# allanbrondum/tfhe-aes-2

Measured on AMD Instinct MI355X. Metric: FHE AES-128 blocks/sec, higher is better.
Workload: dtype f64

## Files before the change

### tfhe-aes-2_amd/csrc/br512x4.hpp

```cpp
#pragma once
#include "br512.hpp"
#include "lf512.hpp"

namespace tae {
namespace br512x4 {

using br512::K1;
using br512::lds_sync;
using br512::M;
using br512::N;
using br512::swap16;
using br512::swap32;
using br512::u32x4;
using br512::wave_sync;

constexpr int C = 3, JOBS = C * K1, THREADS = 1024;

constexpr int BUF_STRIDE = 290;
__device__ constexpr int SF[16] = {-36, -45, -39, -38, -37, -30, -44, -31, -22, -55, -29, -20, -47, -28, -14, -53};
constexpr int SG1[4] = {42, 78, 74, 46};
constexpr int SG3[4] = {13, 81, 157, 225};
__host__ __device__ constexpr int sidx(int q) { return SF[4 * (q & 3) + ((q >> 4) & 3)] + SG1[(q >> 2) & 3] + SG3[q >> 6]; }

#define PRIO(n) __builtin_amdgcn_s_setprio(n)

#ifdef TAE_X4_PROF
#define PROF_DECL uint64_t prof_[10] = {0}, prof_t_ = clock64();
#define PROF_T(i)                        \
    do {                                 \
        asm volatile("" ::: "memory");   \
        const uint64_t now_ = clock64(); \
        prof_[i] += now_ - prof_t_;      \
        prof_t_ = now_;                  \
    } while (0)
#else
#define PROF_DECL
#define PROF_T(i) \
    do {          \
    } while (0)
#endif

constexpr int ACC_STRIDE = N;

#ifdef TAE_X4_HALFTW
__device__ __forceinline__ cplx twmul(cplx a, cplx b) { return {fma(a.re, b.re, a.im), fma(a.im, b.im, a.re)}; }
#else
__device__ __forceinline__ cplx twmul(cplx a, cplx b) { return cmul(a, b); }
#endif

template <bool INV>
__device__ __forceinline__ void dft16x4(cplx *v, const cplx *tw) {
    dft4<INV>(v[0], v[1], v[2], v[3]);
    v[1] = twmul(v[1], INV ? cconj(tw[0]) : tw[0]);
    v[2] = twmul(v[2], INV ? cconj(tw[1]) : tw[1]);
    v[3] = twmul(v[3], INV ? cconj(tw[2]) : tw[2]);
#ifndef TAE_X4_NOSWAP
    swap32(v[0], v[2]);
    swap32(v[1], v[3]);
    swap16(v[0], v[1]);
    swap16(v[2], v[3]);
#endif
    dft4<INV>(v[0], v[1], v[2], v[3]);
}

template <int G>
__device__ __forceinline__ void mac_level(const cplx *buf, int pos, cplx *accr, const cplx *gv) {
    constexpr int PI0 = 4 * G, NA = (15 - PI0) < 4 ? (15 - PI0) : 4, Q0 = PI0 / 3;
#pragma unroll
    for (int p = 0; p < K1; p++) {
        if (p == 2) PRIO(2);
        if (p == 3) PRIO(1);
        if (p == 4) PRIO(0);
        cplx x[C];
#pragma unroll
        for (int c = 0; c < C; c++) x[c] = buf[(c * K1 + p) * BUF_STRIDE + pos];
#pragma unroll
        for (int a = 0; a < NA; a++) {
            const int pi = PI0 + a, q = pi / 3, c = pi % 3;
            const cplx gg = gv[p * 2 + (q - Q0)];
            double re = accr[a].re, im = accr[a].im;
            re = fma(x[c].re, gg.re, re);
            re = fma(-x[c].im, gg.im, re);
            im = fma(x[c].re, gg.im, im);
            im = fma(x[c].im, gg.re, im);
            accr[a] = {re, im};
        }
    }
}

template <int G>
__device__ __forceinline__ void mac_store(cplx *buf, int pos, const cplx *accr) {
    constexpr int PI0 = 4 * G, NA = (15 - PI0) < 4 ? (15 - PI0) : 4;
#pragma unroll
    for (int a = 0; a < NA; a++) {
        const int pi = PI0 + a, q = pi / 3, c = pi % 3;
        buf[(c * K1 + q) * BUF_STRIDE + pos] = accr[a];
    }
}

template <int LEV, bool PBS, int BLOG>
__global__ void __launch_bounds__(THREADS, 1)
    br_kernel(const uint64_t *__restrict__ lwe_in, int n, const uint64_t *__restrict__ lut, int n_out,
              const cplx *__restrict__ ggsw_base, int n_in, uint64_t *__restrict__ out, long B,
              uint64_t body_add, uint64_t out_add, const cplx *__restrict__ twist, const cplx *__restrict__ wtab,
              const double *__restrict__ lf, uint64_t *__restrict__ clk, long lut_mod = 1) {
    constexpr int LOGN = 9;
    ClockStamp stamp;
    stamp.start(clk);
    extern __shared__ __align__(16) unsigned char smem[];
    uint64_t *acc = reinterpret_cast<uint64_t *>(smem);
    cplx *buf = reinterpret_cast<cplx *>(acc + JOBS * ACC_STRIDE);
    cplx *s_tw = buf + JOBS * BUF_STRIDE;
    cplx *s_twa = s_tw + M;
    cplx *s_utw = s_twa + M;
    cplx *s_w16 = s_utw + M;
    double *s_lf = reinterpret_cast<double *>(s_tw);
    const cplx *s_untw = reinterpret_cast<const cplx *>(s_lf + lf512::UNTW);
    const int tid = threadIdx.x;
    const int jb = __builtin_amdgcn_readfirstlane(tid >> 6);
    const int lane = tid & 63, u = lane & 15, r = lane >> 4;
    const bool fjob = jb < JOBS;
    const int jct = fjob ? jb / K1 : 0;
    const size_t ggsw_sz = (size_t)LEV * K1 * K1 * M;

    long ct0, g = 0;
    int nct;
    if (PBS) {
        ct0 = (long)blockIdx.x * C;
        nct = (int)min((long)C, B - ct0);
    } else {
        const int nwg = (int)gridDim.x, q8 = nwg >> 3, r8 = nwg & 7, x8 = (int)blockIdx.x & 7;
        const int lb = x8 * q8 + min(x8, r8) + ((int)blockIdx.x >> 3);
        const int per_group = (n_out + C - 1) / C;
        g = lb / per_group;
        ct0 = (long)(lb - g * per_group) * C;
        nct = min(C, n_out - (int)ct0);
    }
    const bool jvalid = fjob && jct < nct;

    if constexpr (PBS) {
        for (int t = tid; t < lf512::KERNEL_DOUBLES; t += THREADS) s_lf[t] = lf[t];
    } else {
        for (int t = tid; t < M; t += THREADS) {
            s_tw[t] = twist[t];
            s_twa[t] = wtab[(t >> 4) * (t & 15)];
            s_utw[t] = cplx{twist[t].re * 0x1p-8, -twist[t].im * 0x1p-8};
        }
    }
    double lf_s2 = 0, lf_c8 = 0, lf_t8 = 0;
    if constexpr (PBS) {
        lf_s2 = lf[lf512::CONSTS];
        lf_c8 = lf[lf512::CONSTS + 1];
        lf_t8 = lf[lf512::CONSTS + 2];
    }
    if (!PBS && tid < 12) {
        const int rr = tid / 3, k1 = tid - 3 * rr + 1;
        const int e = (rr * k1) & 15;
        const cplx w = wtab[16 * e];
        s_w16[tid] = e == 0 ? cplx{1.0, 0.0} : (e == 4 ? cplx{0.0, -1.0} : w);
    }

    const cplx *gbase = PBS ? ggsw_base : ggsw_base + (size_t)g * n_in * ggsw_sz;
    const uint32_t gbytes = (uint32_t)((size_t)(PBS ? n : n_in) * ggsw_sz * sizeof(cplx));
    const __amdgpu_buffer_rsrc_t grs = __builtin_amdgcn_make_buffer_rsrc((void *)gbase, (short)0, gbytes, 0x00020000);
    const int grp = jb >> 2;
    const int pos = tid & (M - 1);
    const int gvoff = pos * (int)sizeof(cplx);
    const int spos = sidx(pos);
    const int baseA = SF[4 * (u & 3) + r] + SG1[u >> 2], baseB = SF[4 * r + (u & 3)] + SG3[u >> 2];
    const int q0 = (4 * grp) / 3;
    const int nq = grp == 3 ? 1 : 2;

    for (int t = tid; t < JOBS * N; t += THREADS) {
        const int job = t / N, j = t - job * N;
        const int ct = job / K1, c = job - ct * K1;
        uint64_t v = 0;
        if (ct < nct) {
            if (PBS) {
                const uint64_t *in = lwe_in + (size_t)(ct0 + ct) * (n + 1);
                const int bt = mod_switch(in[n] + body_add, LOGN);
                const int e0 = (2 * N - (bt % (2 * N))) % (2 * N);
                v = rotated_coeff(lut + ((ct0 + ct) % lut_mod) * (K1 * N) + c * N, j, e0, N);
            } else {
                v = c < K1 - 1 ? 0 : lut[(size_t)(ct0 + ct) * N + j];
            }
        }
        acc[job * ACC_STRIDE + j] = v;
    }
    lds_sync();

    const int steps = PBS ? n : n_in;
    uint64_t a_next = (PBS && jvalid) ? lwe_in[(size_t)(ct0 + jct) * (n + 1)] : 0;
    cplx accr[4];
    cplx gv[K1 * 2];
    const cplx *my_w16 = s_w16 + 3 * r;
    cplx *jbuf = buf + jb * BUF_STRIDE;
    PROF_DECL
    for (int step = 0; step < steps; step++) {
        int e, gstep;
        if (PBS) {
            const uint64_t a = a_next;
            if (step + 1 < steps && jvalid) a_next = lwe_in[(size_t)(ct0 + jct) * (n + 1) + step + 1];
            e = mod_switch(a, LOGN) % (2 * N);
            gstep = step * (int)(ggsw_sz * sizeof(cplx));
        } else {
            const int b = n_in - 1 - step;
            e = 2 * N - (1 << step);
            gstep = b * (int)(ggsw_sz * sizeof(cplx));
        }
        auto load_level = [&](int lev) {
#pragma unroll
            for (int p = 0; p < K1; p++)
#pragma unroll
                for (int qq = 0; qq < 2; qq++) {
                    if (qq < nq) {
                        const int soff = gstep + (((lev - 1) * K1 + p) * K1 + q0 + qq) * M * (int)sizeof(cplx);
                        const u32x4 rv = __builtin_amdgcn_raw_buffer_load_b128(grs, gvoff, soff, 0);
                        __builtin_memcpy(&gv[p * 2 + qq], &rv, sizeof(cplx));
                    }
                }
        };
        PRIO(3);
        int ll = lane;
        asm volatile("" : "+v"(ll));
        constexpr bool DBYTES = PBS && LEV > 3 && BLOG <= 7;
        uint32_t dig[DBYTES ? (LEV + 1) / 2 : LEV][4];
        constexpr bool FASTDEC = PBS && 128 * LEV * 8 <= (1 << BLOG);
        if (fjob) {
            const uint64_t *poly = acc + jb * ACC_STRIDE;
#pragma unroll
            for (int i = 0; i < 4; i++) {
                const int j = ll + 64 * i;
                uint64_t x0, x1;
                rot_diff<LOGN>(poly, j, e, poly[j], poly[j + M], x0, x1);
                uint32_t dp[LEV];
#ifdef TAE_X4_NODEC
#pragma unroll
                for (int l = 0; l < LEV; l++) dp[l] = (uint32_t)(x0 >> (20 * l)) ^ (uint32_t)(x1 >> (20 * l + 8));
#else
                if constexpr (FASTDEC) {
                    bool dok;
                    decompose16p_fast<LEV, BLOG>(x0, x1, dp, dok);
                    if (__builtin_amdgcn_ballot_w64(!dok)) decompose16p<LEV, BLOG>(x0, x1, dp);
                } else {
                    decompose16p<LEV, BLOG>(x0, x1, dp);
                }
#endif
                if constexpr (DBYTES) {
#pragma unroll
                    for (int l = 0; l < LEV; l += 2) {
                        const uint32_t up = l + 1 < LEV ? dp[(l + 1) % LEV] : 0u;
                        dig[l >> 1][i] = __builtin_amdgcn_perm(up, dp[l], 0x06040200u);
                    }
                } else {
#pragma unroll
                    for (int l = 0; l < LEV; l++) dig[l][i] = dp[l];
                }
            }
        }
#pragma unroll
        for (int a = 0; a < 4; a++) accr[a] = cplx{0.0, 0.0};
        PRIO(2);
        PROF_T(0);

#pragma unroll
        for (int lev = LEV; lev >= 1; lev--) {
            load_level(lev);
            if constexpr (PBS) {
                if (fjob) {
                    cplx v[4];
                    if constexpr (DBYTES) {
                        const int sh = ((lev - 1) & 1) * 16;
                        int dr[4], di[4];
#pragma unroll
                        for (int i = 0; i < 4; i++) {
                            uint32_t dw = dig[0][i];
#pragma unroll
                            for (int w = 1; w < (LEV + 1) / 2; w++)
                                if ((lev - 1) >> 1 == w) dw = dig[w][i];
                            dr[i] = __builtin_amdgcn_sbfe((int)dw, sh, 8);
                            di[i] = __builtin_amdgcn_sbfe((int)dw, sh + 8, 8);
                        }
                        lf512::a1i(dr, di, v, lf_s2, lf_c8, lf_t8);
                    } else {
                        uint32_t dw[4];
#pragma unroll
                        for (int i = 0; i < 4; i++) {
                            dw[i] = dig[0][i];
#pragma unroll
                            for (int l = 1; l < LEV; l++)
                                if (lev - 1 == l) dw[i] = dig[l][i];
                        }
                        lf512::a1(dw, v, lf_s2, lf_c8, lf_t8);
                    }
                    br512::transpose4(v);
                    lf512::dft4<false>(v, lf512::k4(s_lf, lf512::FA2, 4, r));
                    if (lev == LEV) PRIO(2);
#pragma unroll
                    for (int k2 = 0; k2 < 4; k2++) jbuf[baseA + SG3[k2]] = v[k2];
                }
                wave_sync();
                PRIO(1);
                PROF_T(1);
                if (fjob) {
                    cplx v[4];
#pragma unroll
                    for (int i = 0; i < 4; i++) v[i] = jbuf[baseB + SG1[i]];
                    lf512::dft4<false>(v, lf512::k4(s_lf, lf512::FB1, 16, u));
                    br512::transpose4(v);
                    lf512::dft4<false>(v, lf512::k4(s_lf, lf512::FB2, 64, lane));
                    PRIO(0);
#pragma unroll
                    for (int k2 = 0; k2 < 4; k2++) jbuf[baseB + SG1[k2]] = v[k2];
                }
            } else {
            cplx w16[3];
#pragma unroll
            for (int k = 0; k < 3; k++) w16[k] = my_w16[k];
            if (fjob) {
                cplx v[4];
#pragma unroll
                for (int i = 0; i < 4; i++) {
                    uint32_t dw = dig[0][i];
#pragma unroll
                    for (int l = 1; l < LEV; l++)
                        if (lev - 1 == l) dw = dig[l][i];
                    const double a0 = br512::lo16(dw), a1 = br512::hi16(dw);
                    const cplx tw = s_tw[ll + 64 * i];
#ifdef TAE_X4_HALFTW
                    v[i] = {fma(a0, tw.re, a1), fma(a1, tw.im, a0)};
#else
                    v[i] = {fma(a0, tw.re, -(a1 * tw.im)), fma(a0, tw.im, a1 * tw.re)};
#endif
                }
                dft16x4<false>(v, w16);
                if (lev == LEV) PRIO(2);
#pragma unroll
                for (int k2 = 0; k2 < 4; k2++) {
                    const int k = r + 4 * k2;
                    jbuf[baseA + SG3[k2]] = twmul(v[k2], s_twa[16 * k + u]);
                }
            }
            wave_sync();
            PRIO(1);
            PROF_T(1);
            if (fjob) {
                cplx v[4];
#pragma unroll
                for (int i = 0; i < 4; i++) v[i] = jbuf[baseB + SG1[i]];
                dft16x4<false>(v, w16);
                PRIO(0);
#pragma unroll
                for (int k2 = 0; k2 < 4; k2++) jbuf[baseB + SG1[k2]] = v[k2];
            }
            }
            PROF_T(2);
#ifdef TAE_X4_NOBARF
            asm volatile("s_waitcnt lgkmcnt(0)" ::: "memory");
#else
            lds_sync();
#endif
            PROF_T(3);
            PRIO(3);
            switch (grp) {
            case 0: mac_level<0>(buf, spos, accr, gv); break;
            case 1: mac_level<1>(buf, spos, accr, gv); break;
            case 2: mac_level<2>(buf, spos, accr, gv); break;
            default: mac_level<3>(buf, spos, accr, gv); break;
            }
            PROF_T(4);
#ifdef TAE_X4_NOBARM
            if (lev == 1) lds_sync();
#else
            lds_sync();
#endif
            PROF_T(5);
            PRIO(3);
        }
        switch (grp) {
        case 0: mac_store<0>(buf, spos, accr); break;
        case 1: mac_store<1>(buf, spos, accr); break;
        case 2: mac_store<2>(buf, spos, accr); break;
        default: mac_store<3>(buf, spos, accr); break;
        }
        lds_sync();
        PROF_T(6);
        PRIO(3);
        if constexpr (PBS) {
            if (fjob) {
                cplx v[4];
#pragma unroll
                for (int i = 0; i < 4; i++) v[i] = jbuf[baseB + SG1[i]];
                dft4<true>(v[0], v[1], v[2], v[3]);
                br512::transpose4(v);
                lf512::dft4<true>(v, lf512::k4(s_lf, lf512::IB2, 4, r));
#pragma unroll
                for (int k2 = 0; k2 < 4; k2++) jbuf[baseB + SG1[k2]] = v[k2];
            }
            wave_sync();
            PROF_T(7);
            PRIO(3);
            if (fjob) {
                cplx v[4];
#pragma unroll
                for (int i = 0; i < 4; i++) v[i] = jbuf[baseA + SG3[i]];
                lf512::dft4<true>(v, lf512::k4(s_lf, lf512::IA1, 16, u));
                br512::transpose4(v);
                lf512::dft4<true>(v, lf512::k4(s_lf, lf512::IA2, 64, lane));
                uint64_t *poly = acc + jb * ACC_STRIDE;
#pragma unroll
                for (int k2 = 0; k2 < 4; k2++) {
                    const int j = ll + 64 * k2;
                    const cplx t = cmul(v[k2], s_untw[j]);
#ifdef TAE_X4_NOTORUS
                    uint64_t a0 = poly[j] + f64_bits(t.re), a1 = poly[j + M] + f64_bits(t.im);
#else
                    bool o0, o1;
                    uint64_t a0 = torus_add_fast2_sh<8>(t.re, poly[j], o0), a1 = torus_add_fast2_sh<8>(t.im, poly[j + M], o1);
                    if (__builtin_amdgcn_ballot_w64(!(o0 && o1))) {
                        a0 = poly[j] + from_torus_bits(t.re * 0x1p-8);
                        a1 = poly[j + M] + from_torus_bits(t.im * 0x1p-8);
                    }
#endif
                    poly[j] = a0;
                    poly[j + M] = a1;
                }
            }
        } else {
        cplx w16[3];
#pragma unroll
        for (int k = 0; k < 3; k++) w16[k] = my_w16[k];
        if (fjob) {
            cplx v[4];
#pragma unroll
            for (int i = 0; i < 4; i++) v[i] = jbuf[baseB + SG1[i]];
            dft16x4<true>(v, w16);
#pragma unroll
            for (int k2 = 0; k2 < 4; k2++) jbuf[baseB + SG1[k2]] = v[k2];
        }
        wave_sync();
        PROF_T(7);
        PRIO(3);
        if (fjob) {
            cplx v[4];
#pragma unroll
            for (int i = 0; i < 4; i++) {
                const int kk = r + 4 * i;
                v[i] = twmul(jbuf[baseA + SG3[i]], cconj(s_twa[16 * kk + u]));
            }
            dft16x4<true>(v, w16);
            uint64_t *poly = acc + jb * ACC_STRIDE;
#pragma unroll
            for (int k2 = 0; k2 < 4; k2++) {
                const int j = ll + 64 * k2;
                const cplx t = twmul(v[k2], s_utw[j]);
                bool o0, o1;
                uint64_t a0 = torus_add_fast(t.re, poly[j], o0), a1 = torus_add_fast(t.im, poly[j + M], o1);
                if (__builtin_amdgcn_ballot_w64(!(o0 && o1))) {
                    a0 = poly[j] + from_torus_bits(t.re);
                    a1 = poly[j + M] + from_torus_bits(t.im);
                }
                poly[j] = a0;
                poly[j + M] = a1;
            }
        }
        }
        wave_sync();
        PROF_T(8);
#ifdef TAE_X4_PROF
        asm volatile("s_waitcnt lgkmcnt(0)" ::: "memory");
#endif
        PROF_T(9);
    }
#ifdef TAE_X4_PROF
    if (blockIdx.x == 100 && lane == 0)
        printf("x4prof wave %2d: dec %llu passA %llu passB %llu barF %llu mac %llu barM %llu store %llu invB %llu invA %llu end %llu\n",
               jb, (unsigned long long)prof_[0], (unsigned long long)prof_[1], (unsigned long long)prof_[2],
               (unsigned long long)prof_[3], (unsigned long long)prof_[4], (unsigned long long)prof_[5],
               (unsigned long long)prof_[6], (unsigned long long)prof_[7], (unsigned long long)prof_[8],
               (unsigned long long)prof_[9]);
#endif
    lds_sync();
    for (int ct = 0; ct < nct; ct++) {
        const uint64_t *a = acc + ct * K1 * ACC_STRIDE;
        uint64_t *o = PBS ? out + (size_t)(ct0 + ct) * (K1 - 1) * N + (size_t)(ct0 + ct)
                          : out + ((size_t)g * n_out + ct0 + ct) * ((K1 - 1) * N + 1);
        for (int t = tid; t < (K1 - 1) * N; t += THREADS) {
            const int p = t / N, j = t - p * N;
            o[t] = j == 0 ? a[p * ACC_STRIDE] : (0 - a[p * ACC_STRIDE + N - j]);
        }
        if (tid == 0) o[(K1 - 1) * N] = a[(K1 - 1) * ACC_STRIDE] + out_add;
    }
    stamp.stop(clk);
}

inline size_t lds_bytes() {
    return (size_t)JOBS * ACC_STRIDE * 8 + (size_t)JOBS * BUF_STRIDE * 16 + 3 * (size_t)M * 16 + 12 * 16;
}

#define TAE_X4_PARAMS                                                                                         \
    const uint64_t *__restrict__, int, const uint64_t *__restrict__, int, const cplx *__restrict__, int,    \
        uint64_t *__restrict__, long, uint64_t, uint64_t, const cplx *__restrict__, const cplx *__restrict__, \
        const double *__restrict__, uint64_t *__restrict__, long
#ifndef TAE_X4_INSTANTIATE
extern template __global__ void br_kernel<3, true, 12>(TAE_X4_PARAMS);
extern template __global__ void br_kernel<7, true, 6>(TAE_X4_PARAMS);
extern template __global__ void br_kernel<1, false, 13>(TAE_X4_PARAMS);
#endif

}
}
```

Before: 74.47.

## Remap external-product MAC work to per-column ownership with heavy waves for last column

```diff
diff --git a/tfhe-aes-2_amd/csrc/br512x4.hpp b/tfhe-aes-2_amd/csrc/br512x4.hpp
--- a/tfhe-aes-2_amd/csrc/br512x4.hpp
+++ b/tfhe-aes-2_amd/csrc/br512x4.hpp
@@ -95,6 +95,70 @@
     for (int a = 0; a < NA; a++) {
         const int pi = PI0 + a, q = pi / 3, c = pi % 3;
         buf[(c * K1 + q) * BUF_STRIDE + pos] = accr[a];
+    }
+}
+
+__host__ __device__ constexpr int colmap_q(int wave) { return wave >> 2; }
+__host__ __device__ constexpr bool colmap_heavy(int wave) { return (wave & 3) == (wave >> 2); }
+constexpr bool colmap_owns_each_once() {
+    int cnt[K1][M] = {};
+    for (int t = 0; t < THREADS; t++) {
+        cnt[colmap_q(t >> 6)][t & (M - 1)]++;
+        if (colmap_heavy(t >> 6)) cnt[K1 - 1][t & (M - 1)]++;
+    }
+    for (int q = 0; q < K1; q++)
+        for (int pos = 0; pos < M; pos++)
+            if (cnt[q][pos] != 1) return false;
+    return true;
+}
+static_assert(THREADS == (K1 - 1) * M && colmap_owns_each_once(), "every (q, ct, pos) needs exactly one MAC owner");
+template <int LEV, bool PBS>
+constexpr bool COLMAP_FOR =
+#ifdef TAE_X4_COLMAP_ALL
+    true;
+#elif defined(TAE_X4_COLMAP_NONE)
+    false;
+#else
+    PBS && LEV == 7;
+#endif
+
+template <bool HEAVY>
+__device__ __forceinline__ void mac_level_col(const cplx *buf, int pos, cplx *accr, const cplx *gv) {
+#pragma unroll
+    for (int p = 0; p < K1; p++) {
+        if constexpr (!HEAVY) {
+            if (p == 2) PRIO(2);
+            if (p == 3) PRIO(1);
+            if (p == 4) PRIO(0);
+        }
+        cplx x[C];
+#pragma unroll
+        for (int c = 0; c < C; c++) x[c] = buf[(c * K1 + p) * BUF_STRIDE + pos];
+#pragma unroll
+        for (int a = 0; a < (HEAVY ? 2 * C : C); a++) {
+            const int c = a % C;
+            const cplx gg = gv[(a / C) * K1 + p];
+            double re = accr[a].re, im = accr[a].im;
+            re = fma(x[c].re, gg.re, re);
+            re = fma(-x[c].im, gg.im, re);
+            im = fma(x[c].re, gg.im, im);
+            im = fma(x[c].im, gg.re, im);
+            accr[a] = {re, im};
+        }
+    }
+}
+
+template <bool HEAVY>
+__device__ __forceinline__ void mac_store_col(cplx *buf, int pos, int q0, const cplx *accr) {
+    int sq = q0 * BUF_STRIDE;
+    asm volatile("" : "+s"(sq));
+#pragma unroll
+    for (int c = 0; c < C; c++) buf[c * K1 * BUF_STRIDE + sq + pos] = accr[c];
+    if constexpr (HEAVY) {
+        int sl = (K1 - 1) * BUF_STRIDE;
+        asm volatile("" : "+s"(sl));
+#pragma unroll
+        for (int c = 0; c < C; c++) buf[c * K1 * BUF_STRIDE + sl + pos] = accr[C + c];
     }
 }
 
@@ -168,8 +232,10 @@
     const int gvoff = pos * (int)sizeof(cplx);
     const int spos = sidx(pos);
     const int baseA = SF[4 * (u & 3) + r] + SG1[u >> 2], baseB = SF[4 * r + (u & 3)] + SG3[u >> 2];
-    const int q0 = (4 * grp) / 3;
+    constexpr bool COLMAP = COLMAP_FOR<LEV, PBS>;
+    const int q0 = COLMAP ? colmap_q(jb) : (4 * grp) / 3;
     const int nq = grp == 3 ? 1 : 2;
+    const bool heavy = COLMAP && colmap_heavy(jb);
 
     for (int t = tid; t < JOBS * N; t += THREADS) {
         const int job = t / N, j = t - job * N;
@@ -191,7 +257,7 @@
 
     const int steps = PBS ? n : n_in;
     uint64_t a_next = (PBS && jvalid) ? lwe_in[(size_t)(ct0 + jct) * (n + 1)] : 0;
-    cplx accr[4];
+    cplx accr[COLMAP ? 2 * C : 4];
     cplx gv[K1 * 2];
     const cplx *my_w16 = s_w16 + 3 * r;
     cplx *jbuf = buf + jb * BUF_STRIDE;
@@ -208,17 +274,26 @@
             e = 2 * N - (1 << step);
             gstep = b * (int)(ggsw_sz * sizeof(cplx));
         }
+        auto load_row = [&](int lev, int p, int q, cplx &dst) {
+            const int soff = gstep + (((lev - 1) * K1 + p) * K1 + q) * M * (int)sizeof(cplx);
+            const u32x4 rv = __builtin_amdgcn_raw_buffer_load_b128(grs, gvoff, soff, 0);
+            __builtin_memcpy(&dst, &rv, sizeof(cplx));
+        };
         auto load_level = [&](int lev) {
-#pragma unroll
-            for (int p = 0; p < K1; p++)
-#pragma unroll
-                for (int qq = 0; qq < 2; qq++) {
-                    if (qq < nq) {
-                        const int soff = gstep + (((lev - 1) * K1 + p) * K1 + q0 + qq) * M * (int)sizeof(cplx);
-                        const u32x4 rv = __builtin_amdgcn_raw_buffer_load_b128(grs, gvoff, soff, 0);
-                        __builtin_memcpy(&gv[p * 2 + qq], &rv, sizeof(cplx));
-                    }
-                }
+            if constexpr (COLMAP) {
+#pragma unroll
+                for (int p = 0; p < K1; p++) load_row(lev, p, q0, gv[p]);
+                if (heavy) {
+#pragma unroll
+                    for (int p = 0; p < K1; p++) load_row(lev, p, K1 - 1, gv[K1 + p]);
+                }
+            } else {
+#pragma unroll
+                for (int p = 0; p < K1; p++)
+#pragma unroll
+                    for (int qq = 0; qq < 2; qq++)
+                        if (qq < nq) load_row(lev, p, q0 + qq, gv[p * 2 + qq]);
+            }
         };
         PRIO(3);
         int ll = lane;
@@ -259,7 +334,7 @@
             }
         }
 #pragma unroll
-        for (int a = 0; a < 4; a++) accr[a] = cplx{0.0, 0.0};
+        for (int a = 0; a < (COLMAP ? 2 * C : 4); a++) accr[a] = cplx{0.0, 0.0};
         PRIO(2);
         PROF_T(0);
 
@@ -362,11 +437,18 @@
 #endif
             PROF_T(3);
             PRIO(3);
-            switch (grp) {
-            case 0: mac_level<0>(buf, spos, accr, gv); break;
-            case 1: mac_level<1>(buf, spos, accr, gv); break;
-            case 2: mac_level<2>(buf, spos, accr, gv); break;
-            default: mac_level<3>(buf, spos, accr, gv); break;
+            if constexpr (COLMAP) {
+                if (heavy)
+                    mac_level_col<true>(buf, spos, accr, gv);
+                else
+                    mac_level_col<false>(buf, spos, accr, gv);
+            } else {
+                switch (grp) {
+                case 0: mac_level<0>(buf, spos, accr, gv); break;
+                case 1: mac_level<1>(buf, spos, accr, gv); break;
+                case 2: mac_level<2>(buf, spos, accr, gv); break;
+                default: mac_level<3>(buf, spos, accr, gv); break;
+                }
             }
             PROF_T(4);
 #ifdef TAE_X4_NOBARM
@@ -377,11 +459,18 @@
             PROF_T(5);
             PRIO(3);
         }
-        switch (grp) {
-        case 0: mac_store<0>(buf, spos, accr); break;
-        case 1: mac_store<1>(buf, spos, accr); break;
-        case 2: mac_store<2>(buf, spos, accr); break;
-        default: mac_store<3>(buf, spos, accr); break;
+        if constexpr (COLMAP) {
+            if (heavy)
+                mac_store_col<true>(buf, spos, q0, accr);
+            else
+                mac_store_col<false>(buf, spos, q0, accr);
+        } else {
+            switch (grp) {
+            case 0: mac_store<0>(buf, spos, accr); break;
+            case 1: mac_store<1>(buf, spos, accr); break;
+            case 2: mac_store<2>(buf, spos, accr); break;
+            default: mac_store<3>(buf, spos, accr); break;
+            }
         }
         lds_sync();
         PROF_T(6);
@@ -474,11 +563,11 @@
     }
 #ifdef TAE_X4_PROF
     if (blockIdx.x == 100 && lane == 0)
-        printf("x4prof wave %2d: dec %llu passA %llu passB %llu barF %llu mac %llu barM %llu store %llu invB %llu invA %llu end %llu\n",
+        printf("x4prof wave %2d: dec %llu passA %llu passB %llu barF %llu mac %llu barM %llu store %llu invB %llu invA %llu end %llu simd %u\n",
                jb, (unsigned long long)prof_[0], (unsigned long long)prof_[1], (unsigned long long)prof_[2],
                (unsigned long long)prof_[3], (unsigned long long)prof_[4], (unsigned long long)prof_[5],
                (unsigned long long)prof_[6], (unsigned long long)prof_[7], (unsigned long long)prof_[8],
-               (unsigned long long)prof_[9]);
+               (unsigned long long)prof_[9], __builtin_amdgcn_s_getreg((1 << 11) | (4 << 6) | 4));
 #endif
     lds_sync();
     for (int ct = 0; ct < nct; ct++) {
```

After: 74.44 (median of 4 runs). About the same (-0.0%).
